# zhouyifan233/light-transport

Hardware: AMD Instinct MI355X
Metric: photon_steps_per_sec (higher is better)
Workload: dtype f64

## Files before the change

light_transport_amd/csrc/lt_device.hpp:

```cpp
#pragma once
#include <hip/hip_runtime.h>
#include <type_traits>

#define ROCRAND_DETAIL_BM_NOT_IN_STATE
#include <rocrand/rocrand_xorwow.h>
#include <rocrand/rocrand_uniform.h>

#include "lt_internal.hpp"

static_assert(sizeof(rocrand_state_xorwow) == 6 * sizeof(uint32_t), "rocrand_state_xorwow is not {d, x[5]}: SurvD::rng and the tail-split hand-over assume it");

namespace ltk {

#define LT_DEV __device__ __forceinline__
#define LT_PV(name, k) (sizeof(R) == 8 ? (R)P.name[k] : (R)P.f32.name[k])
#define LT_GV(name, k) (sizeof(R) == 8 ? (R)G.name[k] : (R)G.name##32[k])

template <typename R> LT_DEV R sub_rounded(R a, R b)
{
#pragma clang fp contract(off)
    return a - b;
}
#ifdef LT_K_IN_SGPR
LT_DEV double fma_k(double a, double b, double k) { double r; asm("v_fma_f64 %0, %1, %2, %3" : "=v"(r) : "v"(a), "v"(b), "s"(k)); return r; }
// ... 196 lines not shown
    const unsigned j = ((nm >> (sh - 1u)) + 1u) >> 1;
    return *reinterpret_cast<const double2*>(T + 2 * ((int)j - 96));
}
LT_DEV double neg_log_raw(unsigned k, const double2 Tj)
{
    const unsigned n = k + 1u;
    const int lz = __clz((int)n);
    const unsigned nm = n << (lz & 31);
    const unsigned hi = nm >= 0xC0000000u ? 1u : 0u;
    const unsigned sh = 24u + hi;
    const unsigned j = ((nm >> (sh - 1u)) + 1u) >> 1;
    const int dint = (int)(nm - (j << sh));
    const double d = __builtin_ldexp((double)dint, -(int)sh);
    const double r = d * Tj.x;
    double p = 1.0 / 7.0;
    p = fma_k(p, r, -1.0 / 6.0); p = fma_k(p, r, 1.0 / 5.0); p = fma_k(p, r, -0.25); p = fma_k(p, r, 1.0 / 3.0);
    p = __builtin_fma(p, r, -0.5);
    const double lnm = Tj.y + __builtin_fma(r * r, p, r);
    const double de = (double)((int)hi - 1 - lz);
    const double v = -fma_mk(de, 6.93147180369123816490e-01, fma_mk(de, 1.90821492927058770002e-10, lnm));
    return n == 0u ? 0.0 : v;
}
LT_DEV double neg_log_raw(unsigned k, const double* T) { return neg_log_raw(k, neg_log_cell(k, T)); }
LT_DEV double2 sincos_turn_cell(unsigned k, const double* T)
{
    const unsigned iq = (((k + 1u) >> 25) + 1u) >> 1;
    return *reinterpret_cast<const double2*>(T + 2 * (kLnTabEntries + (int)(iq & (unsigned)(kScTabEntries - 1))));
}
LT_DEV void sincos_turn_raw(unsigned k, const double2 Ti, double* sn, double* cs)
{
    const unsigned n = k + 1u;
    const unsigned iq = ((n >> 25) + 1u) >> 1;
    const int drem = (int)(n - (iq << 26));
    const double a = mul_k((double)drem, 1.4629180792671596e-09);
    const double z = a * a;
    double ps = -1.9841269841269841270e-04;
    ps = fma_k(ps, z, 8.3333333333333333333e-03);
    ps = fma_k(ps, z, -1.6666666666666666667e-01);
    const double sd = __builtin_fma(a * z, ps, a);
    double pc = 2.4801587301587301587e-05;
    pc = fma_k(pc, z, -1.3888888888888888889e-03);
    pc = fma_k(pc, z, 4.1666666666666666667e-02);
    pc = __builtin_fma(pc, z, -0.5);
    const double cd = __builtin_fma(pc, z, 1.0);
    *sn = __builtin_fma(Ti.x, cd, Ti.y * sd);
    *cs = __builtin_fma(Ti.y, cd, -(Ti.x * sd));
}
LT_DEV void sincos_turn_raw(unsigned k, const double* T, double* sn, double* cs) { sincos_turn_raw(k, sincos_turn_cell(k, T), sn, cs); }
template <typename R> struct Mx;
template <> struct Mx<double> {
    static LT_DEV double log(double x) { return ::log(x); }
    static LT_DEV double sqrt(double x) { return ::sqrt(x); }
    static LT_DEV double abs(double x) { return ::fabs(x); }
    static LT_DEV double clamp_unit(double c) { return __builtin_fmax(__builtin_fmin(c, 1.0), -1.0); }
    static LT_DEV double sin(double x) { return ::sin(x); }
    static LT_DEV double cos(double x) { return ::cos(x); }
    static LT_DEV double neg_log(double xi, const double* T) { return neg_log_tab(xi, T); }
    static LT_DEV double sqrt_unit(double x) { return sqrt01(x); }
    static LT_DEV double max0(double x) { return __builtin_fmax(x, 0.0); }
    static LT_DEV unsigned sign_word(double x) { return (unsigned)__double2hiint(x); }
    static LT_DEV double max_tiny(double x) { return __builtin_fmax(x, 1e-300); }
    static LT_DEV double sqrt_pos(double x) { return ltk::sqrt_pos(x); }
    static LT_DEV double rsqrt_pos(double x) { return ltk::rsqrt_pos(x); }
    static LT_DEV double quot(double a, double b) { return fast_div(a, b); }
    static LT_DEV double rcp48(double d) { double r = __builtin_amdgcn_rcp(d); return __builtin_fma(__builtin_fma(-d, r, 1.0), r, r); }
    static LT_DEV void sincos_turn(double xi, const double* T, double* s, double* c) { sincos_turn_tab(xi, T, s, c); }
    static LT_DEV double inf() { return __builtin_huge_val(); }
    static LT_DEV double uniform(rocrand_state_xorwow* st)
    {
        const unsigned v1 = rocrand(st), v2 = rocrand(st);
        return fma_kk((double)(((unsigned long long)(v2 >> 11) << 32) | v1), 1.1102230246251565404e-16);
    }
    static LT_DEV double uniform32(rocrand_state_xorwow* st) { return fma_kk((double)rocrand(st), 2.3283064365386962891e-10); }
};
template <> struct Mx<float> {
    static LT_DEV float log(float x) { return ::logf(x); }
    static LT_DEV float sqrt(float x) { return ::sqrtf(x); }
    static LT_DEV float abs(float x) { return ::fabsf(x); }
    static LT_DEV float clamp_unit(float c) { return __builtin_fmaxf(__builtin_fminf(c, 1.0f), -1.0f); }
    static LT_DEV float sin(float x) { return ::sinf(x); }
    static LT_DEV float cos(float x) { return ::cosf(x); }
    static LT_DEV float neg_log(float xi, const double*) { return -::logf(xi); }
    static LT_DEV float sqrt_unit(float x) { return ::sqrtf(__builtin_fmaxf(x, 0.0f)); }
    static LT_DEV float max0(float x) { return __builtin_fmaxf(x, 0.0f); }
    static LT_DEV unsigned sign_word(float x) { return __float_as_uint(x); }
    static LT_DEV float max_tiny(float x) { return __builtin_fmaxf(x, 1e-30f); }
    static LT_DEV float sqrt_pos(float x) { return ::sqrtf(x); }
    static LT_DEV float rsqrt_pos(float x) { return 1.0f / ::sqrtf(x); }
    static LT_DEV float quot(float a, float b) { return a / b; }
    static LT_DEV float rcp48(float d) { return 1.0f / d; }
    static LT_DEV void sincos_turn(float xi, const double*, float* s, float* c) { ::sincospif(2.0f * xi, s, c); }
    static LT_DEV float inf() { return __builtin_huge_valf(); }
    static LT_DEV float uniform(rocrand_state_xorwow* st) { return rocrand_uniform(st); }
    static LT_DEV float uniform32(rocrand_state_xorwow* st) { return rocrand_uniform(st); }
};

template <typename R> LT_DEV R dot3(const R* a, const R* b) { return a[0] * b[0] + a[1] * b[1] + a[2] * b[2]; }
template <typename R> LT_DEV void cross3(const R* a, const R* b, R* o)
{
    o[0] = a[1] * b[2] - a[2] * b[1];
    o[1] = a[2] * b[0] - a[0] * b[2];
    o[2] = a[0] * b[1] - a[1] * b[0];
}
template <typename R> LT_DEV void normalize3(R* v)
{
    R l = Mx<R>::sqrt(v[0] * v[0] + v[1] * v[1] + v[2] * v[2]);
    v[0] /= l; v[1] /= l; v[2] /= l;
}

template <typename R>
LT_DEV R tri_hit(const R* o, const R* d, const TriD<R>* T)
{
    const R eps = (R)1e-7;
    const R nan = (R)__builtin_nanf("");
    R n[3] = {T->n[0], T->n[1], T->n[2]};
    R ddn = dot3(d, n);
    if (Mx<R>::abs(ddn) <= eps) return nan;
    R ab[3] = {T->ab[0], T->ab[1], T->ab[2]};
    R ac[3] = {T->ac[0], T->ac[1], T->ac[2]};
    R pvec[3], qvec[3], tvec[3];
    cross3(d, ac, pvec);
    R det = dot3(ab, pvec);
    if (-eps < det && det < eps) return nan;
    R inv_det = (R)1 / det;
    tvec[0] = o[0] - T->a[0]; tvec[1] = o[1] - T->a[1]; tvec[2] = o[2] - T->a[2];
    R u = dot3(tvec, pvec) * inv_det;
    if (u < 0 || u > 1) return nan;
    cross3(tvec, ab, qvec);
    R v = dot3(d, qvec) * inv_det;
    if (v < 0 || u + v > 1) return nan;
    R t = dot3(ac, qvec) * inv_det;
// ... 628 lines not shown
```

light_transport_amd/csrc/lt_walk.hip:

```cpp
#include "lt_device.hpp"
#include "lt_tally.hpp"

namespace ltk {

template <int TALLY, typename R> LT_DEV typename TallyT<TALLY>::type tally_quantum(R dw)
{
    if constexpr (TALLY == LT_TALLY_U64FX) return (unsigned long long)((double)dw * LT_FX_SCALE + 0.5);
    else return (typename TallyT<TALLY>::type)dw;
}

template <int TALLY> LT_DEV void tally_add(void* grid, unsigned idx, typename TallyT<TALLY>::type v)
{
    if constexpr (TALLY == LT_TALLY_NONE) { asm volatile("" ::"v"(idx), "v"(v)); }
    else
        __hip_atomic_fetch_add(reinterpret_cast<typename TallyT<TALLY>::type*>(grid) + idx, v, __ATOMIC_RELAXED,
                               __HIP_MEMORY_SCOPE_AGENT);
}

template <typename R> struct LdsLayout {
    size_t off_cnt, off_frame, off_media, off_zb, off_if, off_lm, off_lay, off_tris, off_nodes, off_links, off_hist, off_march, off_math, total;
    __host__ __device__ LdsLayout(int n_media, int n_layers, int n_tris, int n_nodes, unsigned n_hist = 0, size_t march_bytes = 0)
    {
        auto al = [](size_t x) { return (x + 15) & ~(size_t)15; };
        size_t o = 0;
        off_cnt = o;   o = al(o + 8 * sizeof(double));
        off_frame = o; o = al(o + 15 * sizeof(R));
        off_media = o; o = al(o + (size_t)n_media * sizeof(MedD<R>));
        off_zb = o;    o = al(o + (size_t)(n_layers + 1) * sizeof(R));
        off_if = o;    o = al(o + (size_t)(n_layers > 0 ? n_layers + 1 : 0) * sizeof(IfD<R>));
        off_lm = o;    o = al(o + (size_t)(n_layers > 0 ? n_layers : 1) * sizeof(int32_t));
        off_lay = o;   o = al(o + (size_t)(n_layers > 0 ? n_layers : 0) * sizeof(LayD<R>));
        off_tris = o;  o = al(o + (size_t)n_tris * sizeof(TriD<R>));
        off_nodes = o; o = al(o + (size_t)n_nodes * sizeof(NodeD<R>));
        off_links = o; o = al(o + (size_t)n_nodes * 16 * sizeof(int16_t));
        off_hist = o;  o = al(o + (size_t)n_hist * sizeof(uint32_t));
        off_march = o; o = al(o + march_bytes);
        off_math = o;  o = al(o + (sizeof(R) == 8 ? kWalkMathTabBytes : 0));
        total = o;
    }
};

LT_DEV unsigned long long readlane64(unsigned long long v, int lane)
{
    unsigned lo = __builtin_amdgcn_readlane((unsigned)v, lane);
    unsigned hi = __builtin_amdgcn_readlane((unsigned)(v >> 32), lane);
    return ((unsigned long long)hi << 32) | lo;
}

LT_DEV unsigned mad_u24(unsigned a, unsigned b, unsigned c)
{
    unsigned r;
    asm("v_mad_u32_u24 %0, %1, %2, %3" : "=v"(r) : "v"(a), "s"(b), "v"(c));
    return r;
}

template <typename T> LT_DEV T wave_sum(T v)
{
#pragma unroll
    for (int off = 32; off > 0; off >>= 1) v += __shfl_down(v, off, 64);
    return v;
}

template <typename R>
LT_DEV void record_vertex(const WalkParams& P, unsigned long long rel, unsigned& nv, R px, R py, R pz, R ux, R uy,
                          R uz, R w, int kind, int medium, unsigned step, R gx, R gy, R gz, R pdf_pos, R pdf_dir)
{
    if (nv < P.max_vertices) {
        lt_vertex* v = P.vertices + rel * (unsigned long long)P.max_vertices + nv;
        v->point[0] = (double)px; v->point[1] = (double)py; v->point[2] = (double)pz;
        v->direction[0] = (double)ux; v->direction[1] = (double)uy; v->direction[2] = (double)uz;
        v->g_norm[0] = (double)gx; v->g_norm[1] = (double)gy; v->g_norm[2] = (double)gz;
        v->throughput = (double)w; v->pdf_pos = (double)pdf_pos; v->pdf_dir = (double)pdf_dir;
        v->kind = kind; v->medium = medium; v->step = step; v->pad_ = 0;
        nv++;
        P.vertex_counts[rel] = nv;
    }
}

// ... 62 lines not shown
    } else {
        if (P.log_idx == nullptr) {
            if (has) tally_add<TALLY>(P.grid, idx, val);
            return;
        }
        const unsigned long long m = __ballot(has);
        if (m == 0ull) return;
        const unsigned cnt = (unsigned)__popcll(m);
        if (lg_chunk != kLogExhausted && lg_end - lg_cur < cnt) log_claim(P, lg_cur, lg_end, lg_chunk);
        if (lg_chunk == kLogExhausted) { log_spill<TALLY>(P, idx, val, has, cnt); return; }
        log_append<TALLY>(P, idx, val, has, m, cnt, lg_cur, s_hist);
    }
}

constexpr unsigned kPacket = 64;
#ifndef LT_REFILL_MIN
#define LT_REFILL_MIN 4
#endif
constexpr unsigned kRefillMin = LT_REFILL_MIN;
#ifndef LT_QUERY_MIN
#define LT_QUERY_MIN 8
#endif
constexpr unsigned kQueryMin = LT_QUERY_MIN;
constexpr unsigned kQueryMinGlobal = 48;
#ifndef LT_QUERY_MAX_AGE
#define LT_QUERY_MAX_AGE 8
#endif
constexpr unsigned kQueryMaxAge = LT_QUERY_MAX_AGE;
#ifndef LT_MARCH_DRAIN_MIN
#define LT_MARCH_DRAIN_MIN 8
#endif
constexpr unsigned kMarchDrainMin = LT_MARCH_DRAIN_MIN;

#ifndef LT_F64_WAVES
#define LT_F64_WAVES 4
#endif
#ifndef LT_F64_GLOBAL_WAVES
#define LT_F64_GLOBAL_WAVES 3
#endif
#ifndef LT_F64_SLAB_WAVES
#define LT_F64_SLAB_WAVES 4
#endif
#ifndef LT_F32_WAVES
#define LT_F32_WAVES 5
#endif
#ifndef LT_INV_MODE_SLAB
#define LT_INV_MODE_SLAB 1
#endif
#ifndef LT_INV_MODE_MESH
#define LT_INV_MODE_MESH 2
#endif
#ifndef LT_INV_MODE_MARCH
#define LT_INV_MODE_MARCH 2
#endif
#define LT_INV_MODE LT_INV_MODE_SLAB
#define LT_WALK_NAME walk_kernel
#define LT_WALK_BATCH 0
#include "lt_walk_kernel.inc"
#undef LT_WALK_NAME
#undef LT_WALK_BATCH
#undef LT_INV_MODE
#define LT_INV_MODE LT_INV_MODE_MESH
#define LT_WALK_NAME walk_kernel_q
#define LT_WALK_BATCH 1
#include "lt_walk_kernel.inc"
#undef LT_WALK_NAME
#undef LT_WALK_BATCH
#undef LT_INV_MODE
#define LT_INV_MODE LT_INV_MODE_MARCH
#define LT_WALK_NAME walk_kernel_m
#define LT_WALK_BATCH 2
#include "lt_walk_kernel.inc"
#undef LT_WALK_NAME
#undef LT_WALK_BATCH
#undef LT_INV_MODE

typedef void (*WalkFn)(const WalkParams);

template <typename R, bool TABLE, bool CAPTURE, int PHASE, int ROUTE>
static WalkFn pick_slab(int tally)
{
    constexpr bool kBuilt = (ROUTE == kRouteLog ? !TABLE && !CAPTURE && PHASE != 2 : PHASE != 1) && (PHASE == 0 || (!TABLE && !CAPTURE));
    if constexpr (kBuilt) {
        switch (tally) {
        case LT_TALLY_F32:
            if constexpr (TABLE) return nullptr;
            else return walk_kernel<R, 0, TABLE, LT_TALLY_F32, CAPTURE, PHASE, ROUTE>;
        case LT_TALLY_F64: return walk_kernel<R, 0, TABLE, LT_TALLY_F64, CAPTURE, PHASE, ROUTE>;
        case LT_TALLY_U64FX: return walk_kernel<R, 0, TABLE, LT_TALLY_U64FX, CAPTURE, PHASE, ROUTE>;
        case LT_TALLY_NONE:
            if constexpr (!TABLE && !CAPTURE && PHASE == 0 && ROUTE == kRouteAtomic) return walk_kernel<R, 0, false, LT_TALLY_NONE, false, 0, kRouteAtomic>;
            else return nullptr;
        }
    }
    return nullptr;
}

template <typename R, int GEOM, bool TABLE, bool CAPTURE>
static WalkFn pick_tally(int tally)
{
    switch (tally) {
    case LT_TALLY_F32:
        if constexpr (TABLE) return nullptr;
        else return walk_kernel_q<R, GEOM, TABLE, LT_TALLY_F32, CAPTURE>;
    case LT_TALLY_F64: return walk_kernel_q<R, GEOM, TABLE, LT_TALLY_F64, CAPTURE>;
    case LT_TALLY_U64FX: return walk_kernel_q<R, GEOM, TABLE, LT_TALLY_U64FX, CAPTURE>;
// ... 94 lines not shown
```

light_transport_amd/csrc/lt_walk_kernel.inc:

```
#ifndef LT_MED
#define LT_MED(i) reinterpret_cast<const MedD<R>*>(reinterpret_cast<const unsigned char*>(s_med) + __umul24((unsigned)(i), (unsigned)sizeof(MedD<R>)))
#define LT_LAY(i) reinterpret_cast<const LayD<R>*>(reinterpret_cast<const unsigned char*>(s_lay) + __umul24((unsigned)(i), (unsigned)sizeof(LayD<R>)))
#endif
#ifndef LT_LAY_LATE
#define LT_LAY_LATE 0
#endif
#ifndef LT_TAB_LATE
#define LT_TAB_LATE 0
#endif
#if LT_WALK_BATCH == 0
#define LT_STEP_Y(held, field) (kLayEarly ? held : Yp->field)
#define LT_STEP_ABSORB LT_STEP_Y(absorb, absorb)
#define LT_STEP_DEP LT_STEP_Y(dep, dep)
#define LT_STEP_HG(xi) hg_sample_walk(xi, LT_STEP_Y(hg_2g, two_g), LT_STEP_Y(hg_1mg, one_m_g), LT_STEP_Y(hg_1mg2, one_m_g2), LT_STEP_Y(hg_1pg2, one_p_g2), LT_STEP_Y(hg_i2g, inv_2g))
#define LT_STEP_G (LT_MED(s_lm[cur])->g)
#else
#define LT_STEP_ABSORB Mp->absorb
#define LT_STEP_DEP Mp->dep
#define LT_STEP_HG(xi) hg_sample_walk(xi, Mp)
#define LT_STEP_G (Mp->g)
#endif
#if LT_WALK_BATCH == 0
template <typename R, int GEOM, bool TABLE, int TALLY, bool CAPTURE, int PHASE, int ROUTE>
#elif LT_WALK_BATCH == 1
template <typename R, int GEOM, bool TABLE, int TALLY, bool CAPTURE, int PHASE = 0>
#else
template <typename R, int GEOM, bool TABLE, int TALLY, bool CAPTURE>
#endif
__global__ void __launch_bounds__(256, (sizeof(R) == 8 ? (GEOM == 0 ? LT_F64_SLAB_WAVES : (GEOM == 2 ? LT_F64_GLOBAL_WAVES : LT_F64_WAVES)) : (GEOM == 0 ? LT_F32_WAVES : 4))) LT_WALK_NAME(const WalkParams P)
{
    constexpr bool MESH = GEOM != 0;
    constexpr bool kSlabForm = LT_WALK_BATCH == 0;
    constexpr bool kLean = kSlabForm && !CAPTURE;
#if LT_WALK_BATCH == 2
    constexpr int PHASE = 0;
#endif
#if LT_WALK_BATCH == 0
    constexpr int kRoute = ROUTE;
#define LT_HAS_LOG (ROUTE == kRouteLog)
    static_assert(ROUTE == kRouteAtomic || ROUTE == kRouteLog, "walk_kernel is built per deposit route");
    static_assert((PHASE != 1 || ROUTE == kRouteLog) && (PHASE != 2 || ROUTE == kRouteAtomic), "bulk kernel: log; tail kernel: atomics");
#else
    constexpr int kRoute = kRouteRuntime;
#define LT_HAS_LOG P.log_idx
#endif
#if LT_WALK_PRIO
    __builtin_amdgcn_s_setprio(LT_WALK_PRIO);
#endif
    extern __shared__ __attribute__((aligned(16))) unsigned char lds_raw[];
    const LdsLayout<R> L(P.n_media, P.n_layers, GEOM == 1 ? P.n_tris : 0, GEOM == 1 ? P.n_nodes : 0,
                         LT_HAS_LOG ? P.log_n_hist : 0u, LT_WALK_BATCH == 2 ? 4 * sizeof(MarchWave<R>) : 0);
    uint32_t* s_hist = reinterpret_cast<uint32_t*>(lds_raw + L.off_hist);
    if (LT_HAS_LOG) for (unsigned t = threadIdx.x; t < P.log_n_hist; t += blockDim.x) s_hist[t] = 0;
    double* s_cnt = reinterpret_cast<double*>(lds_raw + L.off_cnt);
    const MedD<R>* s_med = reinterpret_cast<const MedD<R>*>(lds_raw + L.off_media);
    const R* s_zb = reinterpret_cast<const R*>(lds_raw + L.off_zb);
    const int32_t* s_lm = reinterpret_cast<const int32_t*>(lds_raw + L.off_lm);
    [[maybe_unused]] const LayD<R>* s_lay = reinterpret_cast<const LayD<R>*>(lds_raw + L.off_lay);
    const IfD<R>* s_if = reinterpret_cast<const IfD<R>*>(lds_raw + L.off_if);
    const TriD<R>* s_tris = GEOM == 2 ? reinterpret_cast<const TriD<R>*>(P.tris)
                                      : reinterpret_cast<const TriD<R>*>(lds_raw + L.off_tris);
    const NodeD<R>* s_nodes = GEOM == 2 ? reinterpret_cast<const NodeD<R>*>(P.nodes)
                                        : reinterpret_cast<const NodeD<R>*>(lds_raw + L.off_nodes);

    const int16_t* s_links = !MESH || !P.links ? nullptr
                             : (GEOM == 1 ? reinterpret_cast<const int16_t*>(lds_raw + L.off_links) : P.links);
    if (threadIdx.x < 8) s_cnt[threadIdx.x] = 0.0;
    R* s_frame = reinterpret_cast<R*>(lds_raw + L.off_frame);
    if (threadIdx.x == 64 % blockDim.x && P.src_type == LT_SRC_COSINE_QUAD) {
        const R nrm[3] = {(R)P.src_dir[0], (R)P.src_dir[1], (R)P.src_dir[2]};
        R v2[3], v3[3];
        onb(nrm, v2, v3);
#pragma unroll
        for (int k = 0; k < 3; k++) { s_frame[k] = v2[k]; s_frame[3 + k] = v3[k]; }
    }
#if LT_INV_MODE == 2
    const R* s_inv = s_frame + 6;
    if (threadIdx.x == 128 % blockDim.x) {
#pragma unroll
        for (int k = 0; k < 3; k++) { s_frame[6 + k] = LT_PV(origin, k); s_frame[9 + k] = LT_PV(inv_voxel, k); s_frame[12 + k] = LT_PV(fdim, k); }
    }
#endif
    const double* s_math = reinterpret_cast<const double*>(lds_raw + L.off_math);
    if constexpr (sizeof(R) == 8) lds_copy(lds_raw + L.off_math, kWalkMathTab, kWalkMathTabBytes);
    lds_copy(lds_raw + L.off_media, P.media, (size_t)P.n_media * sizeof(MedD<R>));
    if constexpr (!MESH) {
        lds_copy(lds_raw + L.off_zb, P.zb, (size_t)(P.n_layers + 1) * sizeof(R));
        lds_copy(lds_raw + L.off_lm, P.layer_medium, (size_t)P.n_layers * sizeof(int32_t));
        lds_copy(lds_raw + L.off_if, P.ifaces, (size_t)(P.n_layers + 1) * sizeof(IfD<R>));
        lds_copy(lds_raw + L.off_lay, P.layers, (size_t)P.n_layers * sizeof(LayD<R>));
    } else if constexpr (GEOM == 1) {
        lds_copy(lds_raw + L.off_tris, P.tris, (size_t)P.n_tris * sizeof(TriD<R>));
        lds_copy(lds_raw + L.off_nodes, P.nodes, (size_t)P.n_nodes * sizeof(NodeD<R>));
        if (P.links) lds_copy(lds_raw + L.off_links, P.links, (size_t)P.n_nodes * 16 * sizeof(int16_t));
    }
    __syncthreads();

    const R eps = (R)1e-6;
    const R inf = Mx<R>::inf();
    const int lane = threadIdx.x & 63;

    bool alive = false;
    R px = 0, py = 0, pz = 0, ux = 0, uy = 0, uz = 1, w = 0, sleft = 0;
    int cur = 0;
    unsigned step = 0, max_steps = P.max_steps, nv = 0;
    unsigned long long pid = 0, grp = 0;
    rocrand_state_xorwow rng;
    double acc_abs = 0.0, acc_lost = 0.0;
    unsigned long long acc_steps = 0;
    typedef typename TallyT<TALLY>::type TV;
    unsigned pend_idx = kNoVoxel;
    TV pend_val = 0;
    unsigned lg_cur = 0, lg_end = 0, lg_chunk = kNoVoxel;
    typedef typename std::conditional<kSlabForm, unsigned, unsigned long long>::type pk_t;
    unsigned long long pk_base = 0;
    pk_t pk_next = 0, pk_end = 0;
    bool q_done = false;
    bool dumped = false;
#if LT_WALK_BATCH
    bool q_pend = false;
#if LT_WALK_BATCH == 1
    typename HeldU<R, TABLE>::type q_u1 = 0, q_u2 = 0, q_u3 = 0;
#endif
#if LT_WALK_BATCH == 2
    R q_tc = 0;
    bool q_march = false, q_dirty = false, q_bvh = false;
    unsigned mq_n = 0;
    MarchWave<R>* const mw = reinterpret_cast<MarchWave<R>*>(lds_raw + L.off_march) + (threadIdx.x >> 6);
#endif
#if defined(LT_DIAG_MESH)
    unsigned long long dg_iter = 0, dg_alive = 0, dg_prep = 0, dg_wait = 0, dg_trav_it = 0, dg_trav = 0, dg_go = 0, dg_bnd_it = 0, dg_bnd = 0,
                       dg_int_it = 0, dg_int = 0, dg_refill_it = 0, dg_refill = 0, dg_bvh_it = 0, dg_bvh = 0, dg_l4_it = 0, dg_l4 = 0;
    unsigned long long dg_clk_srv = 0, dg_clk_bnd = 0, dg_clk_all = clock64();
    unsigned long long dgm_clk[4] = {0, 0, 0, 0};
#endif
#endif

#if LT_WALK_BATCH == 1
    const unsigned query_min = P.query_min ? P.query_min : (GEOM == 2 ? kQueryMinGlobal : kQueryMin);
    unsigned q_age = 0;
#elif LT_WALK_BATCH == 2
    const unsigned drain_min = P.query_min ? P.query_min : kMarchDrainMin;
#endif
#if LT_INV_MODE == 2
#define gx0 s_inv[0]
#define gy0 s_inv[1]
#define gz0 s_inv[2]
#define ivx s_inv[3]
#define ivy s_inv[4]
#define ivz s_inv[5]
#define fnx s_inv[6]
#define fny s_inv[7]
#define fnz s_inv[8]
#else
    R gx0 = LT_PV(origin, 0), gy0 = LT_PV(origin, 1), gz0 = LT_PV(origin, 2);
    R ivx = LT_PV(inv_voxel, 0), ivy = LT_PV(inv_voxel, 1), ivz = LT_PV(inv_voxel, 2);
    [[maybe_unused]] const R fnx = LT_PV(fdim, 0), fny = LT_PV(fdim, 1), fnz = LT_PV(fdim, 2);
#if LT_INV_MODE == 1
    asm volatile("" : "+v"(gx0), "+v"(gy0), "+v"(gz0), "+v"(ivx), "+v"(ivy), "+v"(ivz));
#endif
#endif

// ... 80 lines not shown
                        cosine_hemi_frame(nrm, v2, v3, wi, u4[2], u4[3], o4);
                    }
                    e_pdf_dir = Mx<R>::abs(o4[0] * nrm[0] + o4[1] * nrm[1] + o4[2] * nrm[2]) * (R)0.3183098861837907;
                    ux = o4[0]; uy = o4[1]; uz = o4[2];
                    px = (R)P.src_pos[0] + u4[0] * (R)P.src_e1[0] + u4[1] * (R)P.src_e2[0] + eps * o4[0];
                    py = (R)P.src_pos[1] + u4[0] * (R)P.src_e1[1] + u4[1] * (R)P.src_e2[1] + eps * o4[1];
                    pz = (R)P.src_pos[2] + u4[0] * (R)P.src_e1[2] + u4[1] * (R)P.src_e2[2] + eps * o4[2];
                } else {
                    px = (R)P.src_pos[0]; py = (R)P.src_pos[1]; pz = (R)P.src_pos[2];
                    ux = (R)P.src_dir[0]; uy = (R)P.src_dir[1]; uz = (R)P.src_dir[2];
                }
                if constexpr (!MESH) {
                    cur = -1;
                    for (int l = 0; l < P.n_layers; l++)
                        if (pz >= s_zb[l] && pz < s_zb[l + 1]) { cur = l; break; }
                    if (cur < 0) {
                        atomicAdd(&s_cnt[CW_ESC_TOP], (double)w); alive = false;
                    } else if (P.src_type == LT_SRC_PENCIL && pz == s_zb[0] && uz > 0) {
                        R n2 = s_med[s_lm[0]].n, n1 = (R)P.n_above;
                        if (n1 != n2) {
                            R d[3] = {ux, uy, uz}, nf[3] = {0, 0, -1}, ct, refr[3];
                            R Rs = boundary(d, nf, n1, n2, &ct, refr);
                            atomicAdd(&s_cnt[CW_SPECULAR], (double)(w * Rs));
                            w -= w * Rs;
                            if (!(w > 0)) alive = false;
                            ux = refr[0]; uy = refr[1]; uz = refr[2];
                        }
                    }
                } else {
                    cur = P.start_medium;
                }
                nv = 0;
                if constexpr (CAPTURE) if (P.vertices) {
                    P.vertex_counts[id] = 0;
                    if (alive) {
                        R pdf_pos = 1;
                        if (P.src_type == LT_SRC_COSINE_QUAD) {
                            const R e1[3] = {(R)P.src_e1[0], (R)P.src_e1[1], (R)P.src_e1[2]}, e2[3] = {(R)P.src_e2[0], (R)P.src_e2[1], (R)P.src_e2[2]};
                            R cr[3]; cross3(e1, e2, cr);
                            pdf_pos = (R)1 / Mx<R>::sqrt(dot3(cr, cr));
                        }
                        record_vertex<R>(P, id, nv, px, py, pz, ux, uy, uz, w, LT_VERTEX_LIGHT, cur, 0u, (R)P.src_dir[0], (R)P.src_dir[1],
                                         (R)P.src_dir[2], pdf_pos, e_pdf_dir);
                    }
                }
                if constexpr (TABLE) {
                    unsigned long long cap = P.table_steps > grp ? P.table_steps - grp : 0ull;
                    if (cap < (unsigned long long)max_steps) max_steps = (unsigned)cap;
                }
            }
            need = __ballot(!alive);
        }
        if constexpr (kLean) if (need == __ballot(true)) break;
        if constexpr (PHASE == 1) {
            if (q_done && pk_next >= pk_end && !dumped) {
                const unsigned long long am = __ballot(alive);
                const unsigned na = (unsigned)__popcll(am);
                if (na != 0u && na <= P.dump_max) {
                    emit_deposit<TALLY, kRoute>(P, pend_idx, pend_val, lg_cur, lg_end, lg_chunk, s_hist);
                    pend_idx = kNoVoxel;
                    const int leader = __ffsll((long long)am) - 1;
                    unsigned base = 0;
                    if (lane == leader) base = __hip_atomic_fetch_add(P.pool_n, na, __ATOMIC_RELAXED, __HIP_MEMORY_SCOPE_AGENT);
                    base = (unsigned)__builtin_amdgcn_readlane((int)base, leader);
                    if (alive) {
                        const unsigned slot = base + __builtin_amdgcn_mbcnt_hi((unsigned)(am >> 32), __builtin_amdgcn_mbcnt_lo((unsigned)am, 0u));
                        if (slot < P.pool_cap) {
                            SurvD<R>& S = reinterpret_cast<SurvD<R>*>(P.pool)[slot];
                            S.p[0] = px; S.p[1] = py; S.p[2] = pz; S.u[0] = ux; S.u[1] = uy; S.u[2] = uz; S.w = w; S.sleft = sleft;
                            S.pid = 0ull; S.cur = cur; S.step = step;
                            __builtin_memcpy(S.rng, &rng, sizeof S.rng);
#if LT_WALK_BATCH == 1
                            if constexpr (!TABLE) {
                                S.q_pend = q_pend ? 1u : 0u;
                                S.held[0] = __builtin_bit_cast(uint32_t, q_u1); S.held[1] = __builtin_bit_cast(uint32_t, q_u2);
                                S.held[2] = __builtin_bit_cast(uint32_t, q_u3);
                                q_pend = false;
                            }
#else
                            S.q_pend = 0u;
#endif
                            alive = false;
                        }
                    }
                    dumped = true;
                    if constexpr (kLean) if (!__any(alive)) break;
                }
            }
        }
        if constexpr (!kLean) if (!__any(alive)) break;

#if LT_WALK_BATCH == 2
        unsigned f_idx = kNoVoxel;
        TV f_val = 0;
        bool go = false;
        R u1 = 0, s = 0, tb = inf;
        typename HeldU<R, TABLE>::type x2 = 0, x3 = 0;
        int hit_tri = -1;
#if defined(LT_DIAG_MESH)
        const long long dgm_t0 = clock64();
        dg_iter++; dg_alive += __popcll(__ballot(alive)); dg_prep += __popcll(__ballot(alive && !q_pend));
#endif
        if (alive && !q_pend) {
            if (step >= max_steps) {
                atomicAdd(&s_cnt[CW_CAPPED], (double)w); alive = false;
            } else {
                step++;
                acc_steps++;
                const float clr = march_clearance<R>(P.mg, px, py, pz);
                const typename HeldU<R, TABLE>::type x0 = HeldU<R, TABLE>::draw(&rng);
                u1 = Mx<R>::uniform32(&rng);
                x2 = HeldU<R, TABLE>::draw(&rng);
                x3 = HeldU<R, TABLE>::draw(&rng);
                grp++;
                const MedD<R>* Mq = LT_MED(cur);
                if (sleft == 0) sleft = HeldU<R, TABLE>::neg_log(x0, s_math);
                s = (Mq->mu_t > 0) ? sleft * Mq->inv_mu_t : inf;
                if (!(s < (R)clr)) {
                    q_pend = true;
                    mw->held[0][lane] = s; mw->held[1][lane] = u1; mw->held[2][lane] = HeldU<R, TABLE>::as_real(x2); mw->held[3][lane] = HeldU<R, TABLE>::as_real(x3);
                    q_tc = clr > 0.0f ? (R)clr : (R)0;
                    q_march = march_enter<R>(P.mg, mw, px, py, pz, ux, uy, uz, s);
                    q_bvh = !q_march; q_dirty = false;
                } else go = true;
            }
        }
        {
            bool full = false;
#if defined(LT_DIAG_MESH)
            const long long dgm_t1 = clock64();
            dgm_clk[0] += dgm_t1 - dgm_t0;
            { const unsigned long long m_ = __ballot(q_march); if (m_) { dg_trav_it++; dg_trav += __popcll(m_); } }
#endif
            if (__any(q_march)) {
                bool heavy = false;
                full = march_round<R>(P.mg, mw, q_march, heavy, q_dirty, q_tc, mq_n);
                q_bvh = q_bvh || heavy;
            }
#if defined(LT_DIAG_MESH)
// ... 132 lines not shown
                    u1 = HeldU<R, TABLE>::get(q_u1); x2 = q_u2; x3 = q_u3;
                    R o[3] = {px, py, pz}, d[3] = {ux, uy, uz}, th;
                    if constexpr (GEOM == 2) {
                        nearest_bvh_walk(s_tris, s_nodes, P.n_nodes, s_links, o, d, s, hit_tri, th);
                    } else {
                    uint4 rec = make_uint4(0u, 0u, 0xffffffffu, 0xffffffffu);
                    if (P.clear) {
                        const R cx = (px - LT_PV(corg, 0)) * LT_PV(cinv, 0), cy = (py - LT_PV(corg, 1)) * LT_PV(cinv, 1),
                                cz = (pz - LT_PV(corg, 2)) * LT_PV(cinv, 2);
                        if (cx >= 0 && cx < LT_PV(cdim, 0) && cy >= 0 && cy < LT_PV(cdim, 1) && cz >= 0 && cz < LT_PV(cdim, 2))
                            rec = P.clear[((size_t)(int)cz * P.cny + (int)cy) * P.cnx + (int)cx];
                    }
#if defined(LT_DIAG_MESH)
                    {
                        const float c2_ = (float)__builtin_bit_cast(_Float16, (unsigned short)(rec.y & 0xffffu));
                        const float c4_ = (float)__builtin_bit_cast(_Float16, (unsigned short)(rec.y >> 16));
                        const unsigned long long fb = __ballot(!(s < (R)c4_)), f4 = __ballot(!(s < (R)c2_) && s < (R)c4_);
                        if (fb) { dg_bvh_it++; dg_bvh += __popcll(fb); }
                        if (f4) { dg_l4_it++; dg_l4 += __popcll(f4); }
                    }
#endif
                    nearest_listed(s_tris, s_nodes, P.n_nodes, s_links, rec, o, d, s, hit_tri, th);
                    }
                    if (hit_tri >= 0) tb = th;
                    q_pend = false; go = true;
                }
#if defined(LT_DIAG_MESH)
                dg_clk_srv += clock64() - dg_t0;
#endif
            }
        }
#if defined(LT_DIAG_MESH)
        {
            const unsigned long long gm = __ballot(go), bm = __ballot(go && hit_tri >= 0);
            dg_go += __popcll(gm);
            if (bm) { dg_bnd_it++; dg_bnd += __popcll(bm); }
            if (gm & ~bm) { dg_int_it++; dg_int += __popcll(gm & ~bm); }
        }
#endif
#if defined(LT_DIAG_MESH)
        const long long dg_t1 = clock64();
#endif
        if (go) {
            {
                const MedD<R>* Mp = LT_MED(MESH ? cur : s_lm[cur]);
                const R mu_t = Mp->mu_t;
#else
        unsigned f_idx = kNoVoxel;
        TV f_val;
        if constexpr (kLean) asm volatile("" : "=v"(f_val)); else f_val = 0;
        if (alive) {
            if (step >= max_steps) {
                atomicAdd(&s_cnt[CW_CAPPED], (double)w); alive = false;
            } else {
                step++;
                acc_steps++;
                float clr = -1.0f;
                if constexpr (GEOM == 2) {
                    if (P.mg.cell) clr = march_clearance<R>(P.mg, px, py, pz);
                } else if constexpr (MESH) {
                    if (P.clear) {
                        const R cx = (px - LT_PV(corg, 0)) * LT_PV(cinv, 0), cy = (py - LT_PV(corg, 1)) * LT_PV(cinv, 1),
                                cz = (pz - LT_PV(corg, 2)) * LT_PV(cinv, 2);
                        if (cx >= 0 && cx < LT_PV(cdim, 0) && cy >= 0 && cy < LT_PV(cdim, 1) && cz >= 0 && cz < LT_PV(cdim, 2))
                            clr = __uint_as_float(P.clear[((size_t)(int)cz * P.cny + (int)cy) * P.cnx + (int)cx].x);
                    }
                }
                R u1;
                typename HeldU<R, TABLE>::type x0, x2, x3;
                if constexpr (TABLE) {
                    const double* t = P.table + ((pid - P.photon_offset) * P.table_steps + grp) * 4;
                    x0 = (R)(1.0 - t[0]); u1 = (R)(1.0 - t[1]); x2 = (R)(1.0 - t[2]); x3 = (R)(1.0 - t[3]);
                } else {
                    x0 = HeldU<R, TABLE>::draw(&rng);
                    u1 = Mx<R>::uniform32(&rng);
                    x2 = HeldU<R, TABLE>::draw(&rng);
                    x3 = HeldU<R, TABLE>::draw(&rng);
                }
                grp++;
                static_assert(!MESH, "walk_kernel is the slab walk");
                constexpr bool kLayEarly = PHASE != 2 && !CAPTURE && !LT_LAY_LATE;
                constexpr bool kTabEarly = !TABLE && sizeof(R) == 8 && PHASE != 2 && !CAPTURE && !LT_TAB_LATE;
                [[maybe_unused]] const MedD<R>* Mp = s_med;
                const LayD<R>* Yp = LT_LAY(cur);
                const R mu_t = Yp->mu_t, inv_mu_t = Yp->inv_mu_t, z_lo = Yp->z_lo, z_hi = Yp->z_hi;
                [[maybe_unused]] R absorb = 0, dep = 0, hg_2g = 0, hg_1mg = 0, hg_1mg2 = 0, hg_1pg2 = 0, hg_i2g = 0;
                [[maybe_unused]] double2 Tln, Tsc;
                if constexpr (kTabEarly) { Tln = neg_log_cell(x0, s_math); Tsc = sincos_turn_cell(x2, s_math); }
                if constexpr (kLayEarly) {
                    absorb = Yp->absorb; dep = Yp->dep;
                    hg_2g = Yp->two_g; hg_1mg = Yp->one_m_g; hg_1mg2 = Yp->one_m_g2; hg_1pg2 = Yp->one_p_g2; hg_i2g = Yp->inv_2g;
                }
                if constexpr (kLayEarly || kTabEarly) asm volatile("" ::: "memory");
                if (sleft == 0) {
                    if constexpr (kTabEarly) sleft = neg_log_raw(x0, Tln); else sleft = HeldU<R, TABLE>::neg_log(x0, s_math);
                }
                const R s = (mu_t > 0) ? sleft * inv_mu_t : inf;

                R tb = inf; int hit_tri = -1;
                if constexpr (!MESH) {
                    if (uz != 0) {
                        const R dz = (uz > 0 ? z_hi : z_lo) - pz;
                        const R guard = sizeof(R) == 8 ? (R)(1.0 + 1e-12) : (R)(1.0 + 1e-5);
                        const bool near = !(Mx<R>::abs(dz) > s * Mx<R>::abs(uz) * guard);
                        if (__any(near)) {
                            R den = uz;
                            asm volatile("" : "+v"(den));
                            if (near) tb = dz / den;
                        }
                    }
                } else {
                    const bool query = !(s < (R)clr);
                    if (query) {
                        R o[3] = {px, py, pz}, d[3] = {ux, uy, uz}, th;
                        nearest_bvh_walk(s_tris, s_nodes, P.n_nodes, s_links, o, d, s, hit_tri, th);
                        if (hit_tri >= 0) tb = th;
                    }
                }
#endif
                const bool at_boundary = MESH ? (hit_tri >= 0) : (tb <= s);
                if (!at_boundary && !(s < inf)) {
                    atomicAdd(&s_cnt[MESH ? CW_ESC_MESH : CW_CAPPED], (double)w); alive = false;
                } else if (at_boundary) {
                    px += ux * tb; py += uy * tb; pz += uz * tb;
                    sleft -= tb * mu_t;
                    if (!(sleft > 0)) sleft = 0;
                    if constexpr (!MESH) {
                        const bool down = uz > 0;
                        const int k = down ? cur + 1 : cur, next = down ? cur + 1 : cur - 1;
                        pz = s_zb[k];
                        const IfD<R> F = s_if[k];
                        const R Nr = down ? F.nr_down : F.nr_up;
                        R ct;
                        const R Rf = boundary_planar(uz, down ? F.n_up : F.n_dn, down ? F.n_dn : F.n_up, Nr, &ct);
                        const bool refl = HeldU<R, TABLE>::get(x3) <= Rf;
                        const bool gone = !refl && (next < 0 || next >= P.n_layers);
                        if constexpr (CAPTURE) if (P.vertices)
                            record_vertex<R>(P, pid - P.photon_offset, nv, px, py, pz, ux, uy, uz, w,
                                             refl ? LT_VERTEX_REFLECTIVE : LT_VERTEX_TRANSMISSIVE, cur, step, (R)0, (R)0, down ? (R)-1 : (R)1, (R)0,
                                             gone ? (R)0 : (refl ? Rf : (R)1 - Rf));
                        if (refl) uz = -uz;
                        else if (gone) { atomicAdd(&s_cnt[next < 0 ? CW_ESC_TOP : CW_ESC_BOT], (double)w); alive = false; }
                        else { ux *= Nr; uy *= Nr; uz = down ? ct : -ct; cur = next; }
                    } else {
                    R nf[3], n1 = Mp->n, n2; int next;
                    {
                        const TriD<R>* T = &s_tris[hit_tri];
                        R tn[3] = {T->n[0], T->n[1], T->n[2]};
                        R d[3] = {ux, uy, uz};
                        R dn = dot3(d, tn);
                        R sg = dn > 0 ? (R)-1 : (R)1;
                        nf[0] = sg * tn[0]; nf[1] = sg * tn[1]; nf[2] = sg * tn[2];
                        next = dn > 0 ? T->med_front : T->med_back;
                        n2 = next >= 0 ? s_med[next].n : n1;
                    }
                    R d[3] = {ux, uy, uz}, ct, refr[3];
                    R Rf = boundary(d, nf, n1, n2, &ct, refr);
                    if constexpr (CAPTURE) if (P.vertices) {
                        const bool refl = HeldU<R, TABLE>::get(x3) <= Rf;
                        const bool leaves = !refl && next < 0;
                        record_vertex<R>(P, pid - P.photon_offset, nv, px, py, pz, ux, uy, uz, w,
                                         refl ? LT_VERTEX_REFLECTIVE : LT_VERTEX_TRANSMISSIVE, cur, step, nf[0], nf[1], nf[2], (R)0,
                                         leaves ? (R)0 : (refl ? Rf : (R)1 - Rf));
                    }
                    if (HeldU<R, TABLE>::get(x3) <= Rf) {
                        R ro[3]; reflect_walk(d, nf, ro);
                        ux = ro[0]; uy = ro[1]; uz = ro[2];
                        px += eps * nf[0]; py += eps * nf[1]; pz += eps * nf[2];
                    } else if (next < 0) {
                        atomicAdd(&s_cnt[CW_ESC_MESH], (double)w); alive = false;
                    } else {
                        ux = refr[0]; uy = refr[1]; uz = refr[2];
                        px -= eps * nf[0]; py -= eps * nf[1]; pz -= eps * nf[2];
                        cur = next;
                    }
                    }
                } else {
                    px += ux * s; py += uy * s; pz += uz * s;
                    sleft = 0;
                    const R dw = w * LT_STEP_ABSORB;
                    if constexpr (CAPTURE) if (P.vertices) {
                        const R ct_c = LT_STEP_HG(u1);
                        record_vertex<R>(P, pid - P.photon_offset, nv, px, py, pz, ux, uy, uz, w, LT_VERTEX_VOLUME, cur, step, (R)0, (R)0, (R)0,
                                         (R)0, (w - dw > 0) ? hg_pdf(-ct_c, LT_STEP_G) : (R)0);
                    }
                    const R fx = (px - gx0) * ivx, fy = (py - gy0) * ivy, fz = (pz - gz0) * ivz;
                    const unsigned vx = (unsigned)(int)fx, vy = (unsigned)(int)fy, vz = (unsigned)(int)fz;
                    bool inside;
                    if constexpr (!MESH) inside = (int)(Mx<R>::sign_word(fx) | Mx<R>::sign_word(fy) | Mx<R>::sign_word(fz)) >= 0 &&
                                                  vx < (unsigned)P.nx && vy < (unsigned)P.ny && vz < (unsigned)P.nz;
                    else inside = fx >= 0 && fx < fnx && fy >= 0 && fy < fny && fz >= 0 && fz < fnz;
                    unsigned idx;
                    if constexpr (kRoute == kRouteAtomic) idx = (vz * (unsigned)P.ny + vy) * (unsigned)P.nx + vx;
                    else {
                        unsigned tile;
                        if constexpr (kSlabForm) tile = mad_u24(mad_u24(vz >> kTileBZ, P.log_nty, vy >> kTileBY), P.log_ntx, vx >> kTileBX);
                        else tile = __umul24(__umul24(vz >> kTileBZ, P.log_nty) + (vy >> kTileBY), P.log_ntx) + (vx >> kTileBX);
                        idx = kRoute == kRouteLog || P.log_idx
                            ? ((tile << kTileShift) | ((vz & 15u) << 10) | ((vy & 31u) << 5) | (vx & 31u))
                            : (vz * (unsigned)P.ny + vy) * (unsigned)P.nx + vx;
                    }
                    const TV q = tally_quantum<TALLY, R>(w * LT_STEP_DEP);
                    const bool same = inside && idx == pend_idx;
                    const bool flush = inside && !same;
                    f_idx = flush ? pend_idx : kNoVoxel; f_val = pend_val;
                    pend_val = same ? pend_val + q : (flush ? q : pend_val);
                    pend_idx = flush ? idx : pend_idx;
                    acc_abs += inside ? (double)dw : 0.0;
                    acc_lost += inside ? 0.0 : (double)dw;
                    w = sub_rounded(w, dw);
                    if (!(w > 0)) alive = false;
                    else {
                        R u[3] = {ux, uy, uz};
#if LT_WALK_BATCH == 0
                        if constexpr (kTabEarly) {
                            R sp, cp; sincos_turn_raw(x2, Tsc, &sp, &cp);
                            spin_turn(u, LT_STEP_HG(u1), sp, cp);
                        } else
#endif
                        spin<R, TABLE>(u, LT_STEP_HG(u1), x2, s_math);
                        ux = u[0]; uy = u[1]; uz = u[2];
                        if (w < (R)1e-4) {
                            if (HeldU<R, TABLE>::get(x3) <= (R)0.1) { atomicAdd(&s_cnt[CW_ROULETTE], -9.0 * (double)w); w *= (R)10; }
                            else { atomicAdd(&s_cnt[CW_ROULETTE], (double)w); alive = false; }
                        }
                    }
                }
            }
        }
#if LT_WALK_BATCH && defined(LT_DIAG_MESH)
        dg_clk_bnd += clock64() - dg_t1;
#endif
        emit_deposit<TALLY, kRoute>(P, f_idx, f_val, lg_cur, lg_end, lg_chunk, s_hist);
    }
    emit_deposit<TALLY, kRoute>(P, pend_idx, pend_val, lg_cur, lg_end, lg_chunk, s_hist);
    if (LT_HAS_LOG && lg_chunk < kLogExhausted && (threadIdx.x & 63) == 0) P.log_fill[lg_chunk] = lg_cur - lg_chunk * kLogChunk;

#if LT_WALK_BATCH && defined(LT_DIAG_MESH)
#if LT_WALK_BATCH == 2
    if (blockIdx.x == 7 && threadIdx.x == 0) {
        const double tot = (double)(clock64() - dg_clk_all);
        printf("[march diag] iterations %llu, cycles per iteration %.0f | alive %.1f, preparing %.1f | share of the wave's time: prepare %.3f, march round %.3f "
               "(in %.3f of iterations, %.1f lanes), drain %.3f (in %.3f of iterations, %.1f items), resolve %.3f, complete %.3f | complete %.1f lanes: "
               "boundary in %.3f of iterations (%.1f lanes), interaction in %.3f (%.1f lanes) | refills %.3f of iterations (%.1f lanes)\n",
               dg_iter, tot / dg_iter, (double)dg_alive / dg_iter, (double)dg_prep / dg_iter, dgm_clk[0] / tot, dgm_clk[1] / tot, (double)dg_trav_it / dg_iter,
               dg_trav_it ? (double)dg_trav / dg_trav_it : 0.0, dgm_clk[2] / tot, (double)dg_bvh_it / dg_iter, dg_bvh_it ? (double)dg_bvh / dg_bvh_it : 0.0,
               dgm_clk[3] / tot, dg_clk_bnd / tot, (double)dg_go / dg_iter, (double)dg_bnd_it / dg_iter, dg_bnd_it ? (double)dg_bnd / dg_bnd_it : 0.0,
               (double)dg_int_it / dg_iter, dg_int_it ? (double)dg_int / dg_int_it : 0.0, (double)dg_refill_it / dg_iter, dg_refill_it ? (double)dg_refill / dg_refill_it : 0.0);
    }
#else
    if (blockIdx.x == 7 && threadIdx.x == 0) {
        const double tot = (double)(clock64() - dg_clk_all);
        printf("[mesh diag] cycles per service %.0f; share of the wave's time: services %.3f, complete-stage %.3f; cycles per iteration %.0f\n",
               dg_trav_it ? (double)dg_clk_srv / dg_trav_it : 0.0, dg_clk_srv / tot, dg_clk_bnd / tot, tot / dg_iter);
    }
#endif
    if (blockIdx.x == 7 && threadIdx.x == 0)
        printf("[mesh diag] iterations %llu | alive %.1f/64 | prepare %.1f | waiting for a query %.1f | traversals: %.3f of iterations, %.1f lanes each | "
               "complete %.1f lanes: boundary in %.3f of iterations (%.1f lanes), interaction in %.3f (%.1f lanes) | refills: %.3f of iterations, %.1f lanes | "
               "services with BVH lanes %.3f of iterations (%.1f lanes), with 4-triangle lanes %.3f (%.1f lanes)\n",
               dg_iter, (double)dg_alive / dg_iter, (double)dg_prep / dg_iter, (double)dg_wait / dg_iter, (double)dg_trav_it / dg_iter,
               dg_trav_it ? (double)dg_trav / dg_trav_it : 0.0, (double)dg_go / dg_iter, (double)dg_bnd_it / dg_iter,
               dg_bnd_it ? (double)dg_bnd / dg_bnd_it : 0.0, (double)dg_int_it / dg_iter, dg_int_it ? (double)dg_int / dg_int_it : 0.0,
               (double)dg_refill_it / dg_iter, dg_refill_it ? (double)dg_refill / dg_refill_it : 0.0,
               (double)dg_bvh_it / dg_iter, dg_bvh_it ? (double)dg_bvh / dg_bvh_it : 0.0, (double)dg_l4_it / dg_iter, dg_l4_it ? (double)dg_l4 / dg_l4_it : 0.0);
#endif
    const double wa = wave_sum(acc_abs), wl = wave_sum(acc_lost);
    const unsigned long long ws = wave_sum(acc_steps);
    if (lane == 0) {
        atomicAdd(&s_cnt[CW_ABSORBED], wa);
        atomicAdd(&s_cnt[CW_LOST], wl);
        __hip_atomic_fetch_add(&P.counters->steps, ws, __ATOMIC_RELAXED, __HIP_MEMORY_SCOPE_AGENT);
    }
    __syncthreads();
    if (LT_HAS_LOG)
        for (unsigned t = threadIdx.x; t < P.log_n_hist; t += blockDim.x)
            if (s_hist[t]) __hip_atomic_fetch_add(&P.log_hist[t * kLogGroups + (blockIdx.x & (kLogGroups - 1))], s_hist[t],
                                                  __ATOMIC_RELAXED, __HIP_MEMORY_SCOPE_AGENT);
    if (PHASE != 2 && blockIdx.x == 0 && threadIdx.x == 8)
        __hip_atomic_fetch_add(&P.counters->photons, P.n_photons, __ATOMIC_RELAXED, __HIP_MEMORY_SCOPE_AGENT);
    if (threadIdx.x < 8)
        __hip_atomic_fetch_add(&P.counters->w[threadIdx.x], s_cnt[threadIdx.x], __ATOMIC_RELAXED,
                               __HIP_MEMORY_SCOPE_AGENT);
}
#undef LT_HAS_LOG
#undef LT_STEP_ABSORB
#if LT_WALK_BATCH == 0
#undef LT_STEP_Y
#endif
#undef LT_STEP_DEP
#undef LT_STEP_HG
#undef LT_STEP_G
#if LT_INV_MODE == 2
#undef gx0
#undef gy0
#undef gz0
#undef ivx
#undef ivy
#undef ivz
#undef fnx
#undef fny
#undef fnz
#endif
```

Baseline: 96.69 billion.

## Trim per-step register and VALU work in f64 slab walk kernel

Cuts per-lane work in the f64 slab walk loop. Step counting moves to a wave-level scalar popcount of the ballot, with capped photons subtracted afterwards through an LDS counter. Grid dimensions are read from an LDS slot instead of kernel parameters. The voxel tally update uses an FMA with masked accumulation, and the boundary test becomes a flag set where the plane distance is computed. Together these aim to lower VGPR pressure and instruction count, at the cost of fragile LDS aliasing inside the frame block and extra asm barriers.

```diff
diff --git a/light_transport_amd/csrc/lt_device.hpp b/light_transport_amd/csrc/lt_device.hpp
--- a/light_transport_amd/csrc/lt_device.hpp
+++ b/light_transport_amd/csrc/lt_device.hpp
@@ -272,6 +272,7 @@
     static LT_DEV double log(double x) { return ::log(x); }
     static LT_DEV double sqrt(double x) { return ::sqrt(x); }
     static LT_DEV double abs(double x) { return ::fabs(x); }
+    static LT_DEV double fma(double a, double b, double c) { return __builtin_fma(a, b, c); }
     static LT_DEV double clamp_unit(double c) { return __builtin_fmax(__builtin_fmin(c, 1.0), -1.0); }
     static LT_DEV double sin(double x) { return ::sin(x); }
     static LT_DEV double cos(double x) { return ::cos(x); }
@@ -297,6 +298,7 @@
     static LT_DEV float log(float x) { return ::logf(x); }
     static LT_DEV float sqrt(float x) { return ::sqrtf(x); }
     static LT_DEV float abs(float x) { return ::fabsf(x); }
+    static LT_DEV float fma(float a, float b, float c) { return __builtin_fmaf(a, b, c); }
     static LT_DEV float clamp_unit(float c) { return __builtin_fmaxf(__builtin_fminf(c, 1.0f), -1.0f); }
     static LT_DEV float sin(float x) { return ::sinf(x); }
     static LT_DEV float cos(float x) { return ::cosf(x); }
diff --git a/light_transport_amd/csrc/lt_walk.hip b/light_transport_amd/csrc/lt_walk.hip
--- a/light_transport_amd/csrc/lt_walk.hip
+++ b/light_transport_amd/csrc/lt_walk.hip
@@ -19,11 +19,13 @@
 
 template <typename R> struct LdsLayout {
     size_t off_cnt, off_frame, off_media, off_zb, off_if, off_lm, off_lay, off_tris, off_nodes, off_links, off_hist, off_march, off_math, total;
+    static constexpr size_t kCntBytes = 8 * sizeof(double), kFrame = (kCntBytes + 15) & ~(size_t)15;
+    static constexpr size_t kSlabDim = kFrame + 48, kSlabCap = kFrame + (sizeof(R) == 8 ? 64 : 32);
     __host__ __device__ LdsLayout(int n_media, int n_layers, int n_tris, int n_nodes, unsigned n_hist = 0, size_t march_bytes = 0)
     {
         auto al = [](size_t x) { return (x + 15) & ~(size_t)15; };
         size_t o = 0;
-        off_cnt = o;   o = al(o + 8 * sizeof(double));
+        off_cnt = o;   o = al(o + kCntBytes);
         off_frame = o; o = al(o + 15 * sizeof(R));
         off_media = o; o = al(o + (size_t)n_media * sizeof(MedD<R>));
         off_zb = o;    o = al(o + (size_t)(n_layers + 1) * sizeof(R));
@@ -192,6 +194,12 @@
 #endif
 #ifndef LT_INV_MODE_MARCH
 #define LT_INV_MODE_MARCH 2
+#endif
+#ifndef LT_DIET_SIGN32
+#define LT_DIET_SIGN32 1
+#endif
+#ifndef LT_DIET_MASKSUM
+#define LT_DIET_MASKSUM 1
 #endif
 #define LT_INV_MODE LT_INV_MODE_SLAB
 #define LT_WALK_NAME walk_kernel
diff --git a/light_transport_amd/csrc/lt_walk_kernel.inc b/light_transport_amd/csrc/lt_walk_kernel.inc
--- a/light_transport_amd/csrc/lt_walk_kernel.inc
+++ b/light_transport_amd/csrc/lt_walk_kernel.inc
@@ -32,6 +32,8 @@
     constexpr bool MESH = GEOM != 0;
     constexpr bool kSlabForm = LT_WALK_BATCH == 0;
     constexpr bool kLean = kSlabForm && !CAPTURE;
+    constexpr bool kDiet = kSlabForm && sizeof(R) == 8;
+    constexpr bool kMaskSum = kDiet && kLean && LT_DIET_MASKSUM != 0;
 #if LT_WALK_BATCH == 2
     constexpr int PHASE = 0;
 #endif
@@ -56,7 +58,9 @@
     const MedD<R>* s_med = reinterpret_cast<const MedD<R>*>(lds_raw + L.off_media);
     const R* s_zb = reinterpret_cast<const R*>(lds_raw + L.off_zb);
     const int32_t* s_lm = reinterpret_cast<const int32_t*>(lds_raw + L.off_lm);
-    [[maybe_unused]] const LayD<R>* s_lay = reinterpret_cast<const LayD<R>*>(lds_raw + L.off_lay);
+    unsigned lay_off = (unsigned)L.off_lay;
+    if constexpr (kDiet && !CAPTURE && PHASE != 2) asm volatile("" : "+v"(lay_off));
+    [[maybe_unused]] const LayD<R>* s_lay = reinterpret_cast<const LayD<R>*>(lds_raw + lay_off);
     const IfD<R>* s_if = reinterpret_cast<const IfD<R>*>(lds_raw + L.off_if);
     const TriD<R>* s_tris = GEOM == 2 ? reinterpret_cast<const TriD<R>*>(P.tris)
                                       : reinterpret_cast<const TriD<R>*>(lds_raw + L.off_tris);
@@ -73,6 +77,20 @@
         onb(nrm, v2, v3);
 #pragma unroll
         for (int k = 0; k < 3; k++) { s_frame[k] = v2[k]; s_frame[3 + k] = v3[k]; }
+    }
+    constexpr bool kDimLds = kDiet && LT_INV_MODE != 2;
+    constexpr bool kStepsScalar = kLean && kDimLds;
+    if constexpr (kDimLds) {
+        typedef LdsLayout<R> LL;
+        static_assert(LL::kSlabDim % 16 == 0 && LL::kSlabDim >= LL::kFrame + 6 * sizeof(R) && LL::kSlabDim + 16 <= ((LL::kFrame + 15 * sizeof(R) + 15) & ~(size_t)15),
+                      "the dimensions: behind the source frame, inside the frame block");
+        static_assert(LL::kSlabCap % 8 == 0 && LL::kSlabCap >= LL::kFrame + 6 * sizeof(R) && LL::kSlabCap + 8 <= LL::kFrame + 15 * sizeof(R) &&
+                      (LL::kSlabCap + 8 <= LL::kSlabDim || LL::kSlabCap >= LL::kSlabDim + 16), "the capped count: likewise, clear of the dimensions");
+        if (threadIdx.x == 128 % blockDim.x) {
+            unsigned* d = reinterpret_cast<unsigned*>(lds_raw + LdsLayout<R>::kSlabDim);
+            d[0] = (unsigned)P.nx; d[1] = (unsigned)P.ny; d[2] = (unsigned)P.nz; d[3] = 0u;
+            *reinterpret_cast<unsigned long long*>(lds_raw + LdsLayout<R>::kSlabCap) = 0ull;
+        }
     }
 #if LT_INV_MODE == 2
     const R* s_inv = s_frame + 6;
@@ -108,6 +126,7 @@
     rocrand_state_xorwow rng;
     double acc_abs = 0.0, acc_lost = 0.0;
     unsigned long long acc_steps = 0;
+    [[maybe_unused]] unsigned long long steps_w = 0;
     typedef typename TallyT<TALLY>::type TV;
     unsigned pend_idx = kNoVoxel;
     TV pend_val = 0;
@@ -294,6 +313,7 @@
             need = __ballot(!alive);
         }
         if constexpr (kLean) if (need == __ballot(true)) break;
+        if constexpr (kStepsScalar) { steps_w += (unsigned)__popcll(__ballot(true) & ~need); asm volatile("" : "+s"(steps_w)); }
         if constexpr (PHASE == 1) {
             if (q_done && pk_next >= pk_end && !dumped) {
                 const unsigned long long am = __ballot(alive);
@@ -326,7 +346,11 @@
                         }
                     }
                     dumped = true;
-                    if constexpr (kLean) if (!__any(alive)) break;
+                    if constexpr (kStepsScalar) {
+                        const unsigned long long left = __ballot(alive);
+                        steps_w -= na - (unsigned)__popcll(left);
+                        if (left == 0ull) break;
+                    } else if constexpr (kLean) if (!__any(alive)) break;
                 }
             }
         }
@@ -565,9 +589,10 @@
         if (alive) {
             if (step >= max_steps) {
                 atomicAdd(&s_cnt[CW_CAPPED], (double)w); alive = false;
+                if constexpr (kStepsScalar) atomicAdd(reinterpret_cast<unsigned long long*>(lds_raw + LdsLayout<R>::kSlabCap), 1ull);
             } else {
                 step++;
-                acc_steps++;
+                if constexpr (!kStepsScalar) acc_steps++;
                 float clr = -1.0f;
                 if constexpr (GEOM == 2) {
                     if (P.mg.cell) clr = march_clearance<R>(P.mg, px, py, pz);
@@ -610,7 +635,9 @@
                 }
                 const R s = (mu_t > 0) ? sleft * inv_mu_t : inf;
 
-                R tb = inf; int hit_tri = -1;
+                R tb; int hit_tri = -1;
+                bool hop_ends_at_plane = false;
+                if constexpr (kDiet && kLean) asm volatile("" : "=v"(tb)); else tb = inf;
                 if constexpr (!MESH) {
                     if (uz != 0) {
                         const R dz = (uz > 0 ? z_hi : z_lo) - pz;
@@ -619,8 +646,10 @@
                         if (__any(near)) {
                             R den = uz;
                             asm volatile("" : "+v"(den));
-                            if (near) tb = dz / den;
+                            if (near) { tb = dz / den; if constexpr (kDiet) hop_ends_at_plane = tb <= s; }
                         }
+                    } else if constexpr (kDiet) {
+                        if (s == inf) { tb = inf; hop_ends_at_plane = true; }
                     }
                 } else {
                     const bool query = !(s < (R)clr);
@@ -630,8 +659,11 @@
                         if (hit_tri >= 0) tb = th;
                     }
                 }
-#endif
+                const bool at_boundary = kDiet ? hop_ends_at_plane : (tb <= s);
+#endif
+#if LT_WALK_BATCH
                 const bool at_boundary = MESH ? (hit_tri >= 0) : (tb <= s);
+#endif
                 if (!at_boundary && !(s < inf)) {
                     atomicAdd(&s_cnt[MESH ? CW_ESC_MESH : CW_CAPPED], (double)w); alive = false;
                 } else if (at_boundary) {
@@ -700,7 +732,12 @@
                     const R fx = (px - gx0) * ivx, fy = (py - gy0) * ivy, fz = (pz - gz0) * ivz;
                     const unsigned vx = (unsigned)(int)fx, vy = (unsigned)(int)fy, vz = (unsigned)(int)fz;
                     bool inside;
-                    if constexpr (!MESH) inside = (int)(Mx<R>::sign_word(fx) | Mx<R>::sign_word(fy) | Mx<R>::sign_word(fz)) >= 0 &&
+                    if constexpr (kDimLds) {
+                        const uint4 gd = *reinterpret_cast<const uint4*>(lds_raw + LdsLayout<R>::kSlabDim);
+                        unsigned sg = Mx<R>::sign_word(fx) | Mx<R>::sign_word(fy) | Mx<R>::sign_word(fz);
+                        if constexpr (LT_DIET_SIGN32 != 0) asm("" : "+v"(sg));
+                        inside = (int)sg >= 0 && vx < gd.x && vy < gd.y && vz < gd.z;
+                    } else if constexpr (!MESH) inside = (int)(Mx<R>::sign_word(fx) | Mx<R>::sign_word(fy) | Mx<R>::sign_word(fz)) >= 0 &&
                                                   vx < (unsigned)P.nx && vy < (unsigned)P.ny && vz < (unsigned)P.nz;
                     else inside = fx >= 0 && fx < fnx && fy >= 0 && fy < fny && fz >= 0 && fz < fnz;
                     unsigned idx;
@@ -717,10 +754,27 @@
                     const bool same = inside && idx == pend_idx;
                     const bool flush = inside && !same;
                     f_idx = flush ? pend_idx : kNoVoxel; f_val = pend_val;
+                    if constexpr (kDiet) {
+                        if constexpr (kMaskSum) {
+                            if (inside) {
+                                const TV base = same ? pend_val : (TV)0;
+                                if constexpr (std::is_same<TV, R>::value) pend_val = Mx<R>::fma(w, LT_STEP_DEP, base); else pend_val = base + q;
+                                pend_idx = idx;
+                                acc_abs += (double)dw;
+                            } else acc_lost += (double)dw;
+                        } else {
+                            const TV base = flush ? (TV)0 : pend_val;
+                            TV t;
+                            if constexpr (std::is_same<TV, R>::value) t = Mx<R>::fma(w, LT_STEP_DEP, base); else t = base + q;
+                            pend_val = inside ? t : pend_val;
+                        }
+                    } else
                     pend_val = same ? pend_val + q : (flush ? q : pend_val);
-                    pend_idx = flush ? idx : pend_idx;
-                    acc_abs += inside ? (double)dw : 0.0;
-                    acc_lost += inside ? 0.0 : (double)dw;
+                    if constexpr (!kMaskSum) {
+                        pend_idx = flush ? idx : pend_idx;
+                        acc_abs += inside ? (double)dw : 0.0;
+                        acc_lost += inside ? 0.0 : (double)dw;
+                    }
                     w = sub_rounded(w, dw);
                     if (!(w > 0)) alive = false;
                     else {
@@ -779,7 +833,8 @@
                (double)dg_bvh_it / dg_iter, dg_bvh_it ? (double)dg_bvh / dg_bvh_it : 0.0, (double)dg_l4_it / dg_iter, dg_l4_it ? (double)dg_l4 / dg_l4_it : 0.0);
 #endif
     const double wa = wave_sum(acc_abs), wl = wave_sum(acc_lost);
-    const unsigned long long ws = wave_sum(acc_steps);
+    unsigned long long ws;
+    if constexpr (kStepsScalar) ws = steps_w; else ws = wave_sum(acc_steps);
     if (lane == 0) {
         atomicAdd(&s_cnt[CW_ABSORBED], wa);
         atomicAdd(&s_cnt[CW_LOST], wl);
@@ -790,6 +845,10 @@
         for (unsigned t = threadIdx.x; t < P.log_n_hist; t += blockDim.x)
             if (s_hist[t]) __hip_atomic_fetch_add(&P.log_hist[t * kLogGroups + (blockIdx.x & (kLogGroups - 1))], s_hist[t],
                                                   __ATOMIC_RELAXED, __HIP_MEMORY_SCOPE_AGENT);
+    if constexpr (kStepsScalar) if (threadIdx.x == 16 % blockDim.x) {
+        const unsigned long long capped = *reinterpret_cast<const unsigned long long*>(lds_raw + LdsLayout<R>::kSlabCap);
+        if (capped) __hip_atomic_fetch_add(&P.counters->steps, 0ull - capped, __ATOMIC_RELAXED, __HIP_MEMORY_SCOPE_AGENT);
+    }
     if (PHASE != 2 && blockIdx.x == 0 && threadIdx.x == 8)
         __hip_atomic_fetch_add(&P.counters->photons, P.n_photons, __ATOMIC_RELAXED, __HIP_MEMORY_SCOPE_AGENT);
     if (threadIdx.x < 8)
```

After: 98.10 billion, median of 6. 1.5% higher.
